# rafifmalikdzaki/Multitask-Bonetumor-yolo

Measured on AMD Instinct MI355X. Metric: images/sec at 640x640 multitask fwd (det+seg+cls) + decode/NMS/masks, higher is better.
Workload: dtype bf16; 1 GPU; configs[1]: batch-16/GPU 640x640 multitask inference (ConvNeXt-T + C2f-BiFPN + Detect/Segment/cls) + decode + per-image NMS(top-100) + mask assembly; random-init weights; batch_per_gpu=16, img=640, parallelism=dp1 (batch sharded, no data-path collective)

## Files before the change

multitask_bonetumor_yolo_amd/build.py:

```python
import os
import subprocess
import sys
from concurrent.futures import ThreadPoolExecutor

HERE = os.path.dirname(os.path.abspath(__file__))
CSRC = os.path.join(HERE, "csrc")
INCLUDE = os.path.join(os.path.dirname(HERE), "include")
LIB = os.path.join(CSRC, "libmtbt_hip.so")
SOURCES = ["conv_igemm.hip", "conv_igemm_bf16.hip", "conv_igemm_bf16_n.hip", "conv_direct_bf16.hip", "conv_igemm_f32.hip", "conv_igemm_f32_n.hip", "conv_direct_f32.hip", "conv_igemm_f16.hip", "conv_igemm_f16_n.hip", "conv_direct_f16.hip", "conv_batch_bf16.hip", "conv_batch_f16.hip", "conv_batch_f32.hip", "dwconv.hip", "dwconv_bf16.hip", "dwconv_f16.hip", "dwconv_f32.hip", "pointwise.hip", "postprocess.hip", "mask_mfma.hip", "mask_frame.hip", "bn_train.hip", "mlp_fused.hip", "upconv_fused.hip", "node_gemm.hip", "pw_stream.hip", "pw_chain.hip", "loss.hip", "mask_loss.hip", "det_loss_tal.hip", "preprocess.hip", "metrics.hip", "optim.hip", "wgrad.hip", "pointwise_bwd.hip", "train_ops.hip", "resample_bwd.hip", "box_eval.hip", "mask_eval.hip", "box_fuse.hip", "mask_vote.hip", "tile_merge.hip", "mask_tiles.hip"]
HIPCC = os.environ.get("HIPCC", "/opt/rocm/bin/hipcc")
FLAGS = ["--offload-arch=gfx950", "-O3", "-std=c++17", "-fPIC", "-I" + INCLUDE, "-I" + CSRC,
         "-fno-gpu-rdc", "-Wno-unused-value"]
if os.environ.get("MTBT_CONV_ABLATION"):
    FLAGS.append("-DMTBT_CONV_ABLATION")


EXTRA_FLAGS = {"postprocess.hip": ["-ffp-contract=off"], "loss.hip": ["-ffp-contract=off"], "mask_loss.hip": ["-ffp-contract=off"], "det_loss_tal.hip": ["-ffp-contract=off"], "preprocess.hip": ["-ffp-contract=off"], "optim.hip": ["-ffp-contract=off"],
               "box_eval.hip": ["-ffp-contract=off"], "mask_frame.hip": ["-ffp-contract=off"], "box_fuse.hip": ["-ffp-contract=off"], "mask_vote.hip": ["-ffp-contract=off"],
               "tile_merge.hip": ["-ffp-contract=off"], "mask_tiles.hip": ["-ffp-contract=off"]}


def _newer(target, deps):
    if not os.path.exists(target):
        return True
    t = os.path.getmtime(target)
    return any(os.path.getmtime(d) > t for d in deps)


def build(force: bool = False, verbose: bool = False) -> str:
    headers = [os.path.join(INCLUDE, "mtbt_hip.h")] + [os.path.join(CSRC, f) for f in os.listdir(CSRC) if f.endswith((".h", ".inc"))]
    jobs = []
    for s in SOURCES:
        src = os.path.join(CSRC, s)
        obj = os.path.join(CSRC, s.replace(".hip", ".o"))
        if force or _newer(obj, [src] + headers):
            jobs.append([HIPCC] + FLAGS + EXTRA_FLAGS.get(s, []) + ["-c", src, "-o", obj])

    def run(cmd):
        if verbose:
            print(" ".join(cmd), flush=True)
        r = subprocess.run(cmd, capture_output=True, text=True)
        if r.returncode != 0:
            raise RuntimeError("hipcc failed:\n" + " ".join(cmd) + "\n" + r.stdout + r.stderr)

    if jobs:
        with ThreadPoolExecutor(max_workers=min(8, len(jobs))) as ex:
            list(ex.map(run, jobs))
    objs = [os.path.join(CSRC, s.replace(".hip", ".o")) for s in SOURCES]
    if force or jobs or _newer(LIB, objs):
        run([HIPCC, "--offload-arch=gfx950", "-shared", "-fPIC", "-o", LIB] + objs)
    return LIB


if __name__ == "__main__":
    print(build(force="--force" in sys.argv, verbose=True))
```

multitask_bonetumor_yolo_amd/csrc/mlp_fused.hip:

```cpp
#include <cstdlib>

#include "common.h"
#include "conv_params.h"
#include "conv_dma.h"
#include "conv_epilogue.h"

namespace {

typedef __bf16 bf16x2_t __attribute__((ext_vector_type(2)));
typedef float f32x2_t __attribute__((ext_vector_type(2)));
__device__ __forceinline__ uint32_t pk_bf16(float a, float b) {
  return __builtin_bit_cast(uint32_t, __builtin_convertvector(f32x2_t{a, b}, bf16x2_t));
}

__device__ __forceinline__ f32x2_t gelu_poly2(f32x2_t x) {
  const f32x2_t xc = f32x2_t{__builtin_amdgcn_fmed3f(x.x, -4.0f, 4.0f), __builtin_amdgcn_fmed3f(x.y, -4.0f, 4.0f)};
  const f32x2_t s = xc * xc;
  auto k = [](float c) { return f32x2_t{c, c}; };
  f32x2_t p = __builtin_elementwise_fma(k(2.1609857e-08f), s, k(-1.5335673e-06f));
  p = __builtin_elementwise_fma(p, s, k(4.6542096e-05f));
  p = __builtin_elementwise_fma(p, s, k(-7.9887325e-04f));
  p = __builtin_elementwise_fma(p, s, k(8.6900834e-03f));
  p = __builtin_elementwise_fma(p, s, k(-6.4366050e-02f));
  p = __builtin_elementwise_fma(p, s, k(3.9770728e-01f));
  return x * __builtin_elementwise_fma(xc, p, k(0.5f));
}

__device__ __forceinline__ int swz4(int row) { return (-(row >> 2)) & 3; }

#ifdef MTBT_MLP_ABLATION
#define MLP_ABL(p, bit) ((p).dbg & (bit))
#else
#define MLP_ABL(p, bit) 0
#endif

#ifndef MTBT_MLP_RESIDENT
#define MTBT_MLP_RESIDENT 0
#endif

struct MlpP {
  const bf16_t* t;
  const bf16_t* w1;
  const float* b1;
  const bf16_t* w2p;
  const bf16_t* res;
  bf16_t* hpre;
  int M;
  int dbg;
  ConvP ep;
};

template <typename HT> __device__ __forceinline__ uint32_t pk2(float a, float b);
template <> __device__ __forceinline__ uint32_t pk2<bf16_t>(float a, float b) { return pk_bf16(a, b); }
template <> __device__ __forceinline__ uint32_t pk2<f16_t>(float a, float b) { return pk_h2(a, b); }
__device__ __forceinline__ int w2_row_channel(int r) {
  const int F = r >> 4, q = (r >> 2) & 3, e = r & 3;
  return 32 * (F >> 1) + 8 * q + 4 * (F & 1) + e;
}
template <typename HT> __device__ __forceinline__ f32x4 unpack4(uint2 r);
template <> __device__ __forceinline__ f32x4 unpack4<bf16_t>(uint2 r) {
  return f32x4{__uint_as_float(r.x << 16), __uint_as_float(r.x & 0xffff0000u), __uint_as_float(r.y << 16), __uint_as_float(r.y & 0xffff0000u)};
}
template <> __device__ __forceinline__ f32x4 unpack4<f16_t>(uint2 r) { return f32x4{h_lo(r.x), h_hi(r.x), h_lo(r.y), h_hi(r.y)}; }

template <int D, int FP, int WPS, typename HT, bool PIPE = false, bool HP = false>
__global__ __launch_bounds__(256, WPS) void mlp_fused_kernel(const MlpP p) {
  constexpr int KS1 = D / 32;
  constexpr int FC = D / 16;
  constexpr int NCH = 4 * D / 32;
  constexpr int PW = FP * 16, P = 4 * PW;
  constexpr int W1B = 32 * D * 2, W2B = D * 64;
  constexpr int STAGE = W1B + W2B;
  constexpr int NDMA = STAGE / 1024, DPW = NDMA / 4;
  static_assert(NDMA % 4 == 0 && W1B % 1024 == 0, "whole wave-instructions");
  constexpr int NBUF = 3;
  static_assert(NCH % NBUF == 0, "chunk loop is unrolled by the stage count");
  constexpr int AFF_OFF = NBUF * STAGE;

  extern __shared__ __attribute__((aligned(16))) char smem[];
  float* aff = reinterpret_cast<float*>(smem + AFF_OFF);
  const int tid = threadIdx.x, lane = tid & 63;
  const int wave = __builtin_amdgcn_readfirstlane(tid >> 6);
  const int lr = lane & 15, lq = lane >> 4;
  const int pbase = blockIdx.x * P + wave * PW;
  stage_affine<D>(p.ep, aff, 0, tid);
  float* b1s = aff + 2 * D;
  for (int c = tid; c < 4 * D; c += 256) b1s[c] = p.b1[c];

  const srd_t w1srd = make_srd(p.w1), w2srd = make_srd(p.w2p);
  const unsigned lds0 = (unsigned)(size_t)(__attribute__((address_space(3))) char*)smem;
  unsigned voff[DPW];
#pragma unroll
  for (int i = 0; i < DPW; ++i) {
    const int inst = i * 4 + wave;
    const int c = inst * 64 + lane;
    if (inst * 1024 < W1B) {
      const int slab = c / 128, r = (c % 128) / 4, q = (c % 4) ^ swz4(r);
      voff[i] = (unsigned)(r * D * 2 + slab * 64 + q * 16);
    } else {
      const int c2 = c - W1B / 16;
      const int r = c2 / 4, q = (c2 % 4) ^ swz4(r);
      voff[i] = (unsigned)(w2_row_channel(r) * 4 * D * 2 + q * 16);
    }
  }
  auto stage = [&](int j, int buf) {
#pragma unroll
    for (int i = 0; i < DPW; ++i) {
      const int inst = i * 4 + wave;
      const unsigned dst = lds0 + buf * STAGE + inst * 1024;
      if (inst * 1024 < W1B) lds_dma16(w1srd, voff[i], j * 32 * D * 2, dst);
      else lds_dma16(w2srd, voff[i], j * 64, dst);
    }
  };

  uint4 tf[FP][KS1];
#pragma unroll
  for (int f = 0; f < FP; ++f) {
    const int pix = pbase + f * 16 + lr;
#pragma unroll
    for (int ks = 0; ks < KS1; ++ks)
      tf[f][ks] = (pix < p.M && !(p.dbg & 64)) ? *reinterpret_cast<const uint4*>(p.t + (long)pix * D + ks * 32 + lq * 8) : uint4{0u, 0u, 0u, 0u};
  }

  f32x4 acc2[FC][FP];
  static_assert(FC % 2 == 0, "fragment pairs");
#pragma unroll
  for (int f = 0; f < FP; ++f) {
    const int pix = pbase + f * 16 + lr;
#pragma unroll
    for (int m = 0; m < FC / 2; ++m) {
      uint4 r = uint4{0u, 0u, 0u, 0u};
      if (p.res && pix < p.M) r = *reinterpret_cast<const uint4*>(p.res + (long)pix * D + m * 32 + lq * 8);
      acc2[2 * m][f] = unpack4<HT>(uint2{r.x, r.y});
      acc2[2 * m + 1][f] = unpack4<HT>(uint2{r.z, r.w});
    }
  }

  int a1off[KS1], a2off;
#pragma unroll
  for (int ks = 0; ks < KS1; ++ks) a1off[ks] = ks * 2048 + lr * 64 + ((lq ^ swz4(lr)) << 4);
  a2off = W1B + lr * 64 + ((lq ^ swz4(lr)) << 4);

  unsigned hpoff[HP ? FP : 1];
  if constexpr (HP) {
#pragma unroll
    for (int f = 0; f < FP; ++f) hpoff[f] = (unsigned)(pbase + f * 16 + lr) * (unsigned)(8 * D) + (unsigned)(lq * 16);
  }
  stage(0, 0);
  stage(1, 1);
#pragma unroll 1
  for (int j = 0; j < NCH; j += NBUF) {
#pragma unroll
    for (int u = 0; u < NBUF; ++u) {
      const int jj = j + u;
      if (jj + 1 < NCH) wait_vm<DPW + (HP ? FP : 0)>(); else wait_vm<0>();
      lds_barrier();
      if (jj + 2 < NCH && !(p.dbg & 8)) stage(jj + 2, (u + 2) % NBUF);
      const char* st = smem + u * STAGE;
      const float4 ba = *reinterpret_cast<const float4*>(b1s + jj * 32 + lq * 4);
      const float4 bb = *reinterpret_cast<const float4*>(b1s + jj * 32 + 16 + lq * 4);
      if constexpr (PIPE) {
        static_assert(FP == 2, "two pixel blocks per wave");
        uint4 hp0, hp1;
        auto gelu_half = [&](const f32x4& hv, const float4& bv, uint32_t& lo, uint32_t& hi, uint32_t& plo, uint32_t& phi) {
          f32x2_t a01 = f32x2_t{hv[0] + bv.x, hv[1] + bv.y}, a23 = f32x2_t{hv[2] + bv.z, hv[3] + bv.w};
          if constexpr (HP) { plo = pk2<HT>(a01.x, a01.y); phi = pk2<HT>(a23.x, a23.y); }
          a01 = gelu_poly2(a01); a23 = gelu_poly2(a23);
          lo = pk2<HT>(a01.x, a01.y); hi = pk2<HT>(a23.x, a23.y);
        };
        uint4 hb0, hb1;
        f32x4 h0a = f32x4{0.f, 0.f, 0.f, 0.f}, h0b = h0a, h1a = h0a, h1b = h0a;
        {
          uint4 wa[KS1];
#pragma unroll
          for (int ks = 0; ks < KS1; ++ks) wa[ks] = *reinterpret_cast<const uint4*>(st + a1off[ks]);
#pragma unroll
          for (int ks = 0; ks < KS1; ++ks) {
            h0a = mfma_16x16x32<HT>(wa[ks], tf[0][ks], h0a);
            h1a = mfma_16x16x32<HT>(wa[ks], tf[1][ks], h1a);
          }
          __builtin_amdgcn_sched_group_barrier(0x100, KS1, 0);
          __builtin_amdgcn_sched_group_barrier(0x008, 2 * KS1, 0);
        }
        __builtin_amdgcn_sched_barrier(0);
#pragma unroll
        for (int e = 0; e < 4; ++e) { asm volatile("" : "+v"(h0a[e])); asm volatile("" : "+v"(h1a[e])); }
        {
          uint4 wb[KS1];
#pragma unroll
          for (int ks = 0; ks < KS1; ++ks) wb[ks] = *reinterpret_cast<const uint4*>(st + a1off[ks] + 1024);
#pragma unroll
          for (int ks = 0; ks < KS1; ++ks) {
            h0b = mfma_16x16x32<HT>(wb[ks], tf[0][ks], h0b);
            h1b = mfma_16x16x32<HT>(wb[ks], tf[1][ks], h1b);
          }
          gelu_half(h0a, ba, hb0.x, hb0.y, hp0.x, hp0.y);
          gelu_half(h1a, ba, hb1.x, hb1.y, hp1.x, hp1.y);
          __builtin_amdgcn_sched_group_barrier(0x100, KS1, 0);
          __builtin_amdgcn_sched_group_barrier(0x006, 8, 0);
#pragma unroll
          for (int g = 0; g < 2 * KS1; ++g) {
            __builtin_amdgcn_sched_group_barrier(0x008, 1, 0);
            __builtin_amdgcn_sched_group_barrier(0x006, 6, 0);
          }
        }
        __builtin_amdgcn_sched_barrier(0);
        gelu_half(h0b, bb, hb0.z, hb0.w, hp0.z, hp0.w);
        gelu_half(h1b, bb, hb1.z, hb1.w, hp1.z, hp1.w);
        if constexpr (HP) {
          if (pbase + lr < p.M) *reinterpret_cast<uint4*>(reinterpret_cast<char*>(p.hpre) + (size_t)(jj * 64) + (size_t)hpoff[0]) = hp0;
          if (pbase + 16 + lr < p.M) *reinterpret_cast<uint4*>(reinterpret_cast<char*>(p.hpre) + (size_t)(jj * 64) + (size_t)hpoff[1]) = hp1;
        }
        constexpr int PD = 4;
        uint4 w2q[PD];
#pragma unroll
        for (int i = 0; i < PD; ++i) w2q[i] = *reinterpret_cast<const uint4*>(st + a2off + i * 1024);
#pragma unroll
        for (int i = 0; i < FC; ++i) {
          const uint4 w2 = w2q[i % PD];
          if (i + PD < FC) w2q[i % PD] = *reinterpret_cast<const uint4*>(st + a2off + (i + PD) * 1024);
          acc2[i][0] = mfma_16x16x32<HT>(w2, hb0, acc2[i][0]);
          acc2[i][1] = mfma_16x16x32<HT>(w2, hb1, acc2[i][1]);
        }
        __builtin_amdgcn_sched_group_barrier(0x100, PD, 0);
        __builtin_amdgcn_sched_group_barrier(0x006, 400, 0);
#pragma unroll
        for (int i = 0; i < FC; ++i) {
          __builtin_amdgcn_sched_group_barrier(0x008, 2, 0);
          __builtin_amdgcn_sched_group_barrier(0x100, 1, 0);
        }
      } else {
      f32x4 h[2][FP];
#pragma unroll
      for (int b = 0; b < 2; ++b)
#pragma unroll
        for (int f = 0; f < FP; ++f) h[b][f] = f32x4{0.f, 0.f, 0.f, 0.f};
      if (!(p.dbg & 4))
#pragma unroll
      for (int ks = 0; ks < KS1; ++ks) {
        const uint4 wa = *reinterpret_cast<const uint4*>(st + a1off[ks]);
        const uint4 wb = *reinterpret_cast<const uint4*>(st + a1off[ks] + 1024);
#pragma unroll
        for (int f = 0; f < FP; ++f) {
          h[0][f] = mfma_16x16x32<HT>(wa, tf[f][ks], h[0][f]);
          h[1][f] = mfma_16x16x32<HT>(wb, tf[f][ks], h[1][f]);
        }
      }
      uint4 hb[FP];
#pragma unroll
      for (int f = 0; f < FP; ++f) {
        f32x2_t a01 = f32x2_t{h[0][f][0] + ba.x, h[0][f][1] + ba.y}, a23 = f32x2_t{h[0][f][2] + ba.z, h[0][f][3] + ba.w};
        f32x2_t c01 = f32x2_t{h[1][f][0] + bb.x, h[1][f][1] + bb.y}, c23 = f32x2_t{h[1][f][2] + bb.z, h[1][f][3] + bb.w};
        if constexpr (HP) {
          if (pbase + f * 16 + lr < p.M)
            *reinterpret_cast<uint4*>(reinterpret_cast<char*>(p.hpre) + (size_t)(jj * 64) + (size_t)hpoff[f]) =
                uint4{pk2<HT>(a01.x, a01.y), pk2<HT>(a23.x, a23.y), pk2<HT>(c01.x, c01.y), pk2<HT>(c23.x, c23.y)};
        }
        if (!(p.dbg & 1)) { a01 = gelu_poly2(a01); a23 = gelu_poly2(a23); c01 = gelu_poly2(c01); c23 = gelu_poly2(c23); }
        hb[f].x = pk2<HT>(a01.x, a01.y); hb[f].y = pk2<HT>(a23.x, a23.y);
        hb[f].z = pk2<HT>(c01.x, c01.y); hb[f].w = pk2<HT>(c23.x, c23.y);
      }
      if (!(p.dbg & 2))
#pragma unroll
      for (int i = 0; i < FC; ++i) {
        const uint4 w2 = *reinterpret_cast<const uint4*>(st + a2off + i * 1024);
#pragma unroll
        for (int f = 0; f < FP; ++f)
          acc2[i][f] = mfma_16x16x32<HT>(w2, hb[f], acc2[i][f]);
      }
      }
    }
  }
  if (p.dbg & 32) { if (acc2[0][0][0] == 123.f) reinterpret_cast<bf16_t*>(p.ep.y)[0] = 0; return; }
  bf16_t* yb = reinterpret_cast<bf16_t*>(p.ep.y);
#pragma unroll
  for (int m = 0; m < FC / 2; ++m) {
    const float4 s0 = *reinterpret_cast<const float4*>(aff + D + m * 32 + lq * 8), s1 = *reinterpret_cast<const float4*>(aff + D + m * 32 + lq * 8 + 4);
#pragma unroll
    for (int f = 0; f < FP; ++f) {
      const int pix = pbase + f * 16 + lr;
      if (pix >= p.M) continue;
      u32x4 o;
      o.x = pk2<HT>(acc2[2 * m][f][0] + s0.x, acc2[2 * m][f][1] + s0.y);
      o.y = pk2<HT>(acc2[2 * m][f][2] + s0.z, acc2[2 * m][f][3] + s0.w);
      o.z = pk2<HT>(acc2[2 * m + 1][f][0] + s1.x, acc2[2 * m + 1][f][1] + s1.y);
      o.w = pk2<HT>(acc2[2 * m + 1][f][2] + s1.z, acc2[2 * m + 1][f][3] + s1.w);
      *reinterpret_cast<u32x4*>(yb + (long)pix * D + m * 32 + lq * 8) = o;
    }
  }
}

template <int D, int FP, int WPS, typename HT, bool PIPE = false, bool HP = false>
int launch_mlp(const MlpP& p, hipStream_t s) {
  constexpr int P = 4 * FP * 16;
  constexpr int STAGE = 32 * D * 2 + D * 64;
  constexpr int lds = 3 * STAGE + 2 * D * 4 + 4 * D * 4;
  static_assert(lds <= 160 * 1024, "LDS");
  const long blocks = ((long)p.M + P - 1) / P;
  if (blocks <= 0 || blocks > 0x7fffffffL) return MTBT_EINVAL;
  if (int rc = mtbt_allow_lds(mlp_fused_kernel<D, FP, WPS, HT, PIPE, HP>, lds)) return rc;
  hipLaunchKernelGGL((mlp_fused_kernel<D, FP, WPS, HT, PIPE, HP>), dim3((unsigned)blocks), dim3(256), lds, s, p);
  MTBT_LAUNCH_CHECK();
  return MTBT_OK;
}


template <int D, typename HT, bool ORD = false, bool HP = false>
__global__ __launch_bounds__(512, 2) void mlp_pair_kernel(const MlpP p) {
  constexpr int FP = 2;
  constexpr int KS1 = D / 32, FCH = D / 32, NCH = 4 * D / 32;
  constexpr int PW = FP * 16, P = 4 * PW;
  constexpr int W1B = 32 * D * 2, W2B = D * 64, STAGE = W1B + W2B;
  constexpr int NDMA = STAGE / 1024, DPW = NDMA / 8;
  static_assert(NDMA % 8 == 0 && W1B % 1024 == 0, "whole wave-instructions per wave");
  constexpr int XCH_OFF = 2 * STAGE, XCH_BYTES = 2 * 4 * 2 * FP * 64 * 8;
  constexpr int AFF_OFF = XCH_OFF + XCH_BYTES;
  extern __shared__ __attribute__((aligned(16))) char smem[];
  float* aff = reinterpret_cast<float*>(smem + AFF_OFF);
  float* b1s = aff + D;
  const int tid = threadIdx.x, lane = tid & 63;
  const int wave = __builtin_amdgcn_readfirstlane(tid >> 6);
  const int g = wave >> 1, hh = wave & 1;
  const int lr = lane & 15, lq = lane >> 4;
  const int pbase = blockIdx.x * P + g * PW;
  for (int c = tid; c < D; c += 512) aff[c] = p.ep.shift[c];
  for (int c = tid; c < 4 * D; c += 512) b1s[c] = p.b1[c];

  const srd_t w1srd = make_srd(p.w1), w2srd = make_srd(p.w2p);
  const unsigned lds0 = (unsigned)(size_t)(__attribute__((address_space(3))) char*)smem;
  unsigned voff[DPW];
#pragma unroll
  for (int i = 0; i < DPW; ++i) {
    const int inst = i * 8 + wave;
    const int c = inst * 64 + lane;
    if (inst * 1024 < W1B) {
      const int slab = c / 128, r = (c % 128) / 4, sl = (c % 4) ^ swz4(r);
      voff[i] = (unsigned)(r * D * 2 + slab * 64 + sl * 16);
    } else {
      const int c2 = c - W1B / 16;
      const int r = c2 / 4, sl = (c2 % 4) ^ swz4(r);
      voff[i] = (unsigned)(w2_row_channel(r) * 4 * D * 2 + sl * 16);
    }
  }
  auto stage = [&](int j, int buf) {
#pragma unroll
    for (int i = 0; i < DPW; ++i) {
      const int inst = i * 8 + wave;
      const unsigned dst = lds0 + buf * STAGE + inst * 1024;
      if (inst * 1024 < W1B) { if (j < NCH) lds_dma16(w1srd, voff[i], j * 32 * D * 2, dst); }
      else { if (j >= 1) lds_dma16(w2srd, voff[i], (j - 1) * 64, dst); }
    }
  };

  uint4 tf[FP][KS1];
  f32x4 acc2[FCH][FP];
#pragma unroll
  for (int f = 0; f < FP; ++f) {
    const int pix = pbase + f * 16 + lr;
#pragma unroll
    for (int ks = 0; ks < KS1; ++ks)
      tf[f][ks] = (pix < p.M && !MLP_ABL(p, 64)) ? *reinterpret_cast<const uint4*>(p.t + (long)pix * D + ks * 32 + lq * 8) : uint4{0u, 0u, 0u, 0u};
#pragma unroll
    for (int m = 0; m < FCH / 2; ++m) {
      uint4 r = uint4{0u, 0u, 0u, 0u};
      if (p.res && pix < p.M) r = *reinterpret_cast<const uint4*>(p.res + (long)pix * D + (hh * FCH / 2 + m) * 32 + lq * 8);
      acc2[2 * m][f] = unpack4<HT>(uint2{r.x, r.y});
      acc2[2 * m + 1][f] = unpack4<HT>(uint2{r.z, r.w});
    }
  }
  int a1off[KS1];
#pragma unroll
  for (int ks = 0; ks < KS1; ++ks) a1off[ks] = ks * 2048 + hh * 1024 + lr * 64 + ((lq ^ swz4(lr)) << 4);
  const int a2off = W1B + (hh * FCH * 16 + lr) * 64 + ((lq ^ swz4(lr)) << 4);
  uint2* const xch = reinterpret_cast<uint2*>(smem + XCH_OFF);
  const int xmine = ((g * 2 + hh) * FP) * 64 + lane, xpeer = ((g * 2 + (1 - hh)) * FP) * 64 + lane;

  auto gemm2 = [&](const char* st, const uint4 (&hb)[FP]) {
    if (MLP_ABL(p, 2)) return;
#pragma unroll
    for (int i = 0; i < FCH; ++i) {
      const uint4 w2 = *reinterpret_cast<const uint4*>(st + a2off + i * 1024);
#pragma unroll
      for (int f = 0; f < FP; ++f) acc2[i][f] = mfma_16x16x32<HT>(w2, hb[f], acc2[i][f]);
    }
  };
  const bool ord = ORD && (wave & 4);
  uint2 mine[FP];
#pragma unroll
  for (int f = 0; f < FP; ++f) mine[f] = uint2{0u, 0u};
  unsigned hpoff[HP ? FP : 1];
  if constexpr (HP) {
#pragma unroll
    for (int f = 0; f < FP; ++f) hpoff[f] = (unsigned)(pbase + f * 16 + lr) * (unsigned)(8 * D) + (unsigned)(lq * 16 + hh * 8);
  }
  stage(0, 0);
#pragma unroll 1
  for (int j0 = 0; j0 <= NCH; j0 += 2) {
#pragma unroll
    for (int u = 0; u < 2; ++u) {
      const int j = j0 + u;
      if (j > NCH) break;
      wait_vm<0>();
      lds_barrier();
      if (j + 1 <= NCH && !MLP_ABL(p, 8)) stage(j + 1, (u + 1) & 1);
      const char* st = smem + u * STAGE;
      uint4 hb[FP];
      if (j >= 1) {
#pragma unroll
        for (int f = 0; f < FP; ++f) {
          const uint2 peer = xch[((u + 1) & 1) * (4 * 2 * FP * 64) + xpeer + f * 64];
          hb[f] = hh == 0 ? uint4{mine[f].x, mine[f].y, peer.x, peer.y} : uint4{peer.x, peer.y, mine[f].x, mine[f].y};
        }
      }
      f32x4 h[FP];
      const bool g2_first = ord && j >= 1;
      if (g2_first) gemm2(st, hb);
      if (j < NCH) {
#pragma unroll
        for (int f = 0; f < FP; ++f) h[f] = f32x4{0.f, 0.f, 0.f, 0.f};
        if (!MLP_ABL(p, 4))
#pragma unroll
        for (int ks = 0; ks < KS1; ++ks) {
          const uint4 w = *reinterpret_cast<const uint4*>(st + a1off[ks]);
#pragma unroll
          for (int f = 0; f < FP; ++f) h[f] = mfma_16x16x32<HT>(w, tf[f][ks], h[f]);
        }
      }
      if (j >= 1 && !g2_first) gemm2(st, hb);
      if (j < NCH) {
        const float4 bv = *reinterpret_cast<const float4*>(b1s + j * 32 + hh * 16 + lq * 4);
#pragma unroll
        for (int f = 0; f < FP; ++f) {
          f32x2_t a01 = f32x2_t{h[f][0] + bv.x, h[f][1] + bv.y}, a23 = f32x2_t{h[f][2] + bv.z, h[f][3] + bv.w};
          if constexpr (HP) {
            if (pbase + f * 16 + lr < p.M)
              *reinterpret_cast<uint2*>(reinterpret_cast<char*>(p.hpre) + (size_t)(j * 64) + (size_t)hpoff[f]) = uint2{pk2<HT>(a01.x, a01.y), pk2<HT>(a23.x, a23.y)};
          }
          if (!MLP_ABL(p, 1)) { a01 = gelu_poly2(a01); a23 = gelu_poly2(a23); }
          mine[f] = uint2{pk2<HT>(a01.x, a01.y), pk2<HT>(a23.x, a23.y)};
          xch[u * (4 * 2 * FP * 64) + xmine + f * 64] = mine[f];
        }
      }
    }
  }
  HT* const yb = reinterpret_cast<HT*>(p.ep.y);
  static_assert(FCH % 2 == 0, "fragment pairs");
#pragma unroll
  for (int m = 0; m < FCH / 2; ++m) {
    const int cb = (hh * FCH / 2 + m) * 32 + lq * 8;
    const float4 s0 = *reinterpret_cast<const float4*>(aff + cb), s1 = *reinterpret_cast<const float4*>(aff + cb + 4);
#pragma unroll
    for (int f = 0; f < FP; ++f) {
      const int pix = pbase + f * 16 + lr;
      if (pix >= p.M || MLP_ABL(p, 32)) continue;
      u32x4 o;
      o.x = pk2<HT>(acc2[2 * m][f][0] + s0.x, acc2[2 * m][f][1] + s0.y);
      o.y = pk2<HT>(acc2[2 * m][f][2] + s0.z, acc2[2 * m][f][3] + s0.w);
      o.z = pk2<HT>(acc2[2 * m + 1][f][0] + s1.x, acc2[2 * m + 1][f][1] + s1.y);
      o.w = pk2<HT>(acc2[2 * m + 1][f][2] + s1.z, acc2[2 * m + 1][f][3] + s1.w);
      *reinterpret_cast<u32x4*>(yb + (long)pix * D + cb) = o;
    }
  }
}

template <int D, typename HT, bool ORD = false, bool HP = false>
int launch_mlp_pair(const MlpP& p, hipStream_t s) {
  constexpr int P = 4 * 2 * 16;
  constexpr int STAGE = 32 * D * 2 + D * 64;
  constexpr int lds = 2 * STAGE + 2 * 4 * 2 * 2 * 64 * 8 + 5 * D * 4;
  static_assert(lds <= 160 * 1024, "LDS");
  const long blocks = ((long)p.M + P - 1) / P;
  if (blocks <= 0 || blocks > 0x7fffffffL) return MTBT_EINVAL;
  if (int rc = mtbt_allow_lds(mlp_pair_kernel<D, HT, ORD, HP>, lds)) return rc;
  hipLaunchKernelGGL((mlp_pair_kernel<D, HT, ORD, HP>), dim3((unsigned)blocks), dim3(512), lds, s, p);
  MTBT_LAUNCH_CHECK();
  return MTBT_OK;
}

template <int D, typename HT, int NW, bool PREF = false>
__global__ __launch_bounds__(NW * 64, NW / 4) void mlp_resident_kernel(const MlpP p) {
  constexpr int FP = 2;
  constexpr int KS1 = D / 32, FC = D / 16, NCH = 4 * D / 32;
  constexpr int W1B = 32 * D * 2, W2B = D * 64, STAGE = W1B + W2B;
  static_assert(NCH * STAGE + 6 * D * 4 <= 160 * 1024, "the weights must fit the LDS");
  extern __shared__ __attribute__((aligned(16))) char smem[];
  float* aff = reinterpret_cast<float*>(smem + NCH * STAGE);
  float* b1s = aff + D;
  const int tid = threadIdx.x, lane = tid & 63;
  const int wave = __builtin_amdgcn_readfirstlane(tid >> 6);
  const int lr = lane & 15, lq = lane >> 4;
  for (int c = tid; c < D; c += NW * 64) aff[c] = p.ep.shift[c];
  for (int c = tid; c < 4 * D; c += NW * 64) b1s[c] = p.b1[c];
  {
    const srd_t w1srd = make_srd(p.w1), w2srd = make_srd(p.w2p);
    const unsigned lds0 = (unsigned)(size_t)(__attribute__((address_space(3))) char*)smem;
    constexpr int NDMA = STAGE / 1024;
    for (int q = wave; q < NCH * NDMA; q += NW) {
      const int j = q / NDMA, inst = q - j * NDMA;
      const int c = inst * 64 + lane;
      unsigned vo;
      if (inst * 1024 < W1B) {
        const int slab = c / 128, r = (c % 128) / 4, sl = (c % 4) ^ swz4(r);
        vo = (unsigned)(r * D * 2 + slab * 64 + sl * 16);
        lds_dma16(w1srd, vo, j * 32 * D * 2, __builtin_amdgcn_readfirstlane(lds0 + j * STAGE + inst * 1024));
      } else {
        const int c2 = c - W1B / 16;
        const int r = c2 / 4, sl = (c2 % 4) ^ swz4(r);
        vo = (unsigned)(r * 4 * D * 2 + sl * 16);
        lds_dma16(w2srd, vo, j * 64, __builtin_amdgcn_readfirstlane(lds0 + j * STAGE + inst * 1024));
      }
    }
    wait_vm<0>();
  }
  __syncthreads();

  int a1off[KS1], a2off;
#pragma unroll
  for (int ks = 0; ks < KS1; ++ks) a1off[ks] = ks * 2048 + lr * 64 + ((lq ^ swz4(lr)) << 4);
  a2off = W1B + lr * 64 + ((lq ^ swz4(lr)) << 4);

  const int nblk = (p.M + 31) / 32;
  const int G = gridDim.x, per_round = G * NW;
  const int rounds = nblk / per_round, rem = nblk - rounds * per_round;
  const int mine = rounds + ((wave * G + (int)blockIdx.x) < rem ? 1 : 0);
  HT* const yb = reinterpret_cast<HT*>(p.ep.y);
  auto block_of = [&](int it) { return it < rounds ? it * per_round + (int)blockIdx.x * NW + wave : rounds * per_round + wave * G + (int)blockIdx.x; };
  auto fetch = [&](int blk, uint4 (&tf_)[FP][KS1], uint2 (&rr_)[FC][FP]) {
#pragma unroll
    for (int f = 0; f < FP; ++f) {
      const int pix = blk * 32 + f * 16 + lr;
#pragma unroll
      for (int ks = 0; ks < KS1; ++ks)
        tf_[f][ks] = (pix < p.M && !MLP_ABL(p, 64)) ? *reinterpret_cast<const uint4*>(p.t + (unsigned)(pix * D + ks * 32 + lq * 8)) : uint4{0u, 0u, 0u, 0u};
#pragma unroll
      for (int i = 0; i < FC; ++i)
        rr_[i][f] = (p.res && pix < p.M) ? *reinterpret_cast<const uint2*>(p.res + (unsigned)(pix * D + i * 16 + lq * 4)) : uint2{0u, 0u};
    }
  };
  uint4 tf[FP][KS1], tfn[FP][KS1];
  uint2 rr[FC][FP], rrn[FC][FP];
  if (PREF && mine > 0) fetch(block_of(0), tf, rr);
#pragma unroll 1
  for (int it = 0; it < mine; ++it) {
    const int blk = block_of(it);
    const int pbase = blk * 32;
    if (PREF) { if (it + 1 < mine) fetch(block_of(it + 1), tfn, rrn); }
    else fetch(blk, tf, rr);
    f32x4 acc2[FC][FP];
#pragma unroll
    for (int f = 0; f < FP; ++f)
#pragma unroll
      for (int i = 0; i < FC; ++i) acc2[i][f] = unpack4<HT>(rr[i][f]);
#pragma unroll 1
    for (int jj = 0; jj < NCH; ++jj) {
      const char* st = smem + jj * STAGE;
      const float4 ba = *reinterpret_cast<const float4*>(b1s + jj * 32 + lq * 4);
      const float4 bb = *reinterpret_cast<const float4*>(b1s + jj * 32 + 16 + lq * 4);
      f32x4 h[2][FP];
#pragma unroll
      for (int b = 0; b < 2; ++b)
#pragma unroll
        for (int f = 0; f < FP; ++f) h[b][f] = f32x4{0.f, 0.f, 0.f, 0.f};
      if (!MLP_ABL(p, 4))
#pragma unroll
      for (int ks = 0; ks < KS1; ++ks) {
        const uint4 wa = *reinterpret_cast<const uint4*>(st + a1off[ks]);
        const uint4 wb = *reinterpret_cast<const uint4*>(st + a1off[ks] + 1024);
#pragma unroll
        for (int f = 0; f < FP; ++f) {
          h[0][f] = mfma_16x16x32<HT>(wa, tf[f][ks], h[0][f]);
          h[1][f] = mfma_16x16x32<HT>(wb, tf[f][ks], h[1][f]);
        }
      }
      uint4 hb[FP];
#pragma unroll
      for (int f = 0; f < FP; ++f) {
        f32x2_t a01 = f32x2_t{h[0][f][0] + ba.x, h[0][f][1] + ba.y}, a23 = f32x2_t{h[0][f][2] + ba.z, h[0][f][3] + ba.w};
        f32x2_t c01 = f32x2_t{h[1][f][0] + bb.x, h[1][f][1] + bb.y}, c23 = f32x2_t{h[1][f][2] + bb.z, h[1][f][3] + bb.w};
        if (!MLP_ABL(p, 1)) { a01 = gelu_poly2(a01); a23 = gelu_poly2(a23); c01 = gelu_poly2(c01); c23 = gelu_poly2(c23); }
        hb[f].x = pk2<HT>(a01.x, a01.y); hb[f].y = pk2<HT>(a23.x, a23.y);
        hb[f].z = pk2<HT>(c01.x, c01.y); hb[f].w = pk2<HT>(c23.x, c23.y);
      }
      if (!MLP_ABL(p, 2))
#pragma unroll
      for (int i = 0; i < FC; ++i) {
        const uint4 w2 = *reinterpret_cast<const uint4*>(st + a2off + i * 1024);
#pragma unroll
        for (int f = 0; f < FP; ++f) acc2[i][f] = mfma_16x16x32<HT>(w2, hb[f], acc2[i][f]);
      }
    }
#pragma unroll
    for (int i = 0; i < FC; ++i) {
      const float4 sh = *reinterpret_cast<const float4*>(aff + i * 16 + lq * 4);
#pragma unroll
      for (int f = 0; f < FP; ++f) {
        const int pix = pbase + f * 16 + lr;
        if (pix >= p.M || MLP_ABL(p, 32)) continue;
        uint2 o;
        o.x = pk2<HT>(acc2[i][f][0] + sh.x, acc2[i][f][1] + sh.y);
        o.y = pk2<HT>(acc2[i][f][2] + sh.z, acc2[i][f][3] + sh.w);
        *reinterpret_cast<uint2*>(yb + (unsigned)(pix * D + i * 16 + lq * 4)) = o;
      }
    }
    if (PREF) {
#pragma unroll
      for (int f = 0; f < FP; ++f) {
#pragma unroll
        for (int ks = 0; ks < KS1; ++ks) tf[f][ks] = tfn[f][ks];
#pragma unroll
        for (int i = 0; i < FC; ++i) rr[i][f] = rrn[i][f];
      }
    }
  }
}

template <int D, typename HT, int NW = 16, bool PREF = false>
int launch_mlp_resident(const MlpP& p, hipStream_t s) {
  constexpr int lds = (4 * D / 32) * (32 * D * 2 + D * 64) + 5 * D * 4;
  const long nblk = ((long)p.M + 31) / 32;
  long blocks = (nblk + NW - 1) / NW;
  if (blocks > 256) blocks = 256;
  if (blocks <= 0) return MTBT_EINVAL;
  if (int rc = mtbt_allow_lds(mlp_resident_kernel<D, HT, NW, PREF>, lds)) return rc;
  hipLaunchKernelGGL((mlp_resident_kernel<D, HT, NW, PREF>), dim3((unsigned)blocks), dim3(NW * 64), lds, s, p);
  MTBT_LAUNCH_CHECK();
  return MTBT_OK;
}

}

static int mlp_entry(const void* t, const void* res, const void* w1, const float* b1, const void* w2p, const float* b2, void* y, int64_t M, int D,
                     int dtype, void* stream, void* hpre = nullptr) {
  if (!t || !w1 || !b1 || !w2p || !b2 || !y || M <= 0 || M > 0x7fffff00L) return MTBT_EINVAL;
  if (hpre && (dtype != MTBT_BF16 || !aligned16(hpre) || M * 8 * (int64_t)D >= 0xffff0000L)) return MTBT_EINVAL;
  if (dtype != MTBT_BF16 && dtype != MTBT_F16) return MTBT_EINVAL;
  if (D != 96 && D != 192 && D != 384) return MTBT_EINVAL;
  if (!aligned16(t) || !aligned16(w1) || !aligned16(w2p) || !aligned16(y) || !aligned16(b1) || (res && !aligned16(res))) return MTBT_EALIGN;
  if ((long)4 * D * D * 2 >= 0x7fff0000L) return MTBT_EINVAL;
  MlpP p;
  p.t = reinterpret_cast<const bf16_t*>(t); p.w1 = reinterpret_cast<const bf16_t*>(w1); p.b1 = b1;
  p.w2p = reinterpret_cast<const bf16_t*>(w2p); p.M = (int)M;
  p.dbg = 0;
  p.hpre = reinterpret_cast<bf16_t*>(hpre);
  ConvP& e = p.ep;
  e = ConvP{};
  p.res = (p.dbg & 16) ? nullptr : reinterpret_cast<const bf16_t*>(res);
  e.y = y; e.res = nullptr;
  e.scale = nullptr; e.shift = b2; e.K = D; e.ldy = D; e.ldr = D; e.act = MTBT_ACT_NONE;
  e.out_mode = MTBT_OUT_NHWC; e.out_f32 = 0; e.vec_ok = 1; e.M = (int)M;
  hipStream_t s = reinterpret_cast<hipStream_t>(stream);
  if (D == 96 && M >= 64 * 1024 && M * 96 < 0x7fffffffL && MTBT_MLP_RESIDENT)
    return dtype == MTBT_F16 ? launch_mlp_resident<96, f16_t, 8, true>(p, s) : launch_mlp_resident<96, bf16_t, 8, true>(p, s);
  if (hpre) {
    if (D == 384) return MTBT_EINVAL;
    if (D == 192) return launch_mlp<192, 2, 2, bf16_t, true, true>(p, s);
    return launch_mlp<96, 2, 4, bf16_t, false, true>(p, s);
  }
  if (D == 384) return dtype == MTBT_F16 ? launch_mlp_pair<384, f16_t>(p, s) : launch_mlp_pair<384, bf16_t>(p, s);
  if (D == 192) return dtype == MTBT_F16 ? launch_mlp<192, 2, 2, f16_t, true>(p, s) : launch_mlp<192, 2, 2, bf16_t, true>(p, s);
  return dtype == MTBT_F16 ? launch_mlp<96, 2, 4, f16_t>(p, s) : launch_mlp<96, 2, 4, bf16_t>(p, s);
}

extern "C" int mtbt_convnext_mlp_fused(const void* t, const void* res, const void* w1, const float* b1, const void* w2p,
                                       const float* b2, void* y, int64_t M, int D, void* stream) {
  return mlp_entry(t, res, w1, b1, w2p, b2, y, M, D, MTBT_BF16, stream);
}

extern "C" int mtbt_convnext_mlp_fused_dt(const void* t, const void* res, const void* w1, const float* b1, const void* w2p,
                                          const float* b2, void* y, int64_t M, int D, int dtype, void* stream) {
  return mlp_entry(t, res, w1, b1, w2p, b2, y, M, D, dtype, stream);
}

extern "C" int mtbt_convnext_mlp_fused_train(const void* t, const void* res, const void* w1_perm, const float* b1_perm, const void* w2, const float* b2,
                                             void* y, void* hpre, int64_t M, int D, void* stream) {
  if (!hpre) return MTBT_EINVAL;
  return mlp_entry(t, res, w1_perm, b1_perm, w2, b2, y, M, D, MTBT_BF16, stream, hpre);
}
```

Before: 2707 images/s.

## Deepen mlp_pair weight ring and interleave GELU with GEMM2 MFMAs

The pair MLP kernel gains a RING=3 default mode in which W1 chunks are triple-buffered and W2' chunks double-buffered in LDS, so staging runs further ahead of compute and uses partial vmcnt waits. GELU is split into staged pieces that are interleaved with the GEMM2 MFMA steps, and LDS weight fragments are prefetched a couple of steps ahead, with sched_barriers pinning the order. The aim is to hide DMA latency and VALU GELU work behind matrix instructions. In exchange it uses more LDS per block, which may reduce occupancy, adds register pressure, and makes the scheduling fragile. The build also compiles a test probe library.

Measured after the change: 2742 images/s (median of 6 runs). Within noise of the previous version (+1.3%).

```diff
diff --git a/multitask_bonetumor_yolo_amd/build.py b/multitask_bonetumor_yolo_amd/build.py
--- a/multitask_bonetumor_yolo_amd/build.py
+++ b/multitask_bonetumor_yolo_amd/build.py
@@ -8,6 +8,8 @@
 INCLUDE = os.path.join(os.path.dirname(HERE), "include")
 LIB = os.path.join(CSRC, "libmtbt_hip.so")
 SOURCES = ["conv_igemm.hip", "conv_igemm_bf16.hip", "conv_igemm_bf16_n.hip", "conv_direct_bf16.hip", "conv_igemm_f32.hip", "conv_igemm_f32_n.hip", "conv_direct_f32.hip", "conv_igemm_f16.hip", "conv_igemm_f16_n.hip", "conv_direct_f16.hip", "conv_batch_bf16.hip", "conv_batch_f16.hip", "conv_batch_f32.hip", "dwconv.hip", "dwconv_bf16.hip", "dwconv_f16.hip", "dwconv_f32.hip", "pointwise.hip", "postprocess.hip", "mask_mfma.hip", "mask_frame.hip", "bn_train.hip", "mlp_fused.hip", "upconv_fused.hip", "node_gemm.hip", "pw_stream.hip", "pw_chain.hip", "loss.hip", "mask_loss.hip", "det_loss_tal.hip", "preprocess.hip", "metrics.hip", "optim.hip", "wgrad.hip", "pointwise_bwd.hip", "train_ops.hip", "resample_bwd.hip", "box_eval.hip", "mask_eval.hip", "box_fuse.hip", "mask_vote.hip", "tile_merge.hip", "mask_tiles.hip"]
+PROBES = os.path.join(os.path.dirname(HERE), "tools", "probes")
+TEST_PROBES = ["mlp_pair_ring"]
 HIPCC = os.environ.get("HIPCC", "/opt/rocm/bin/hipcc")
 FLAGS = ["--offload-arch=gfx950", "-O3", "-std=c++17", "-fPIC", "-I" + INCLUDE, "-I" + CSRC,
          "-fno-gpu-rdc", "-Wno-unused-value"]
@@ -27,8 +29,30 @@
     return any(os.path.getmtime(d) > t for d in deps)
 
 
+def _headers():
+    return [os.path.join(INCLUDE, "mtbt_hip.h")] + [os.path.join(CSRC, f) for f in os.listdir(CSRC) if f.endswith((".h", ".inc"))]
+
+
+def _probe_job(name, force):
+    src = os.path.join(PROBES, name + ".hip")
+    lib = os.path.join(PROBES, "lib" + name + ".so")
+    deps = [src] + _headers() + [os.path.join(CSRC, f) for f in os.listdir(CSRC) if f.endswith(".hip")]
+    cmd = [HIPCC] + FLAGS + ["-shared", src, "-o", lib] if force or _newer(lib, deps) else None
+    return lib, cmd
+
+
+def build_probe(name: str, force: bool = False) -> str:
+    lib, cmd = _probe_job(name, force)
+    if cmd:
+        r = subprocess.run(cmd, capture_output=True, text=True)
+        if r.returncode != 0:
+            raise RuntimeError("hipcc failed:\n" + " ".join(cmd) + "\n" + r.stdout + r.stderr)
+    return lib
+
+
 def build(force: bool = False, verbose: bool = False) -> str:
-    headers = [os.path.join(INCLUDE, "mtbt_hip.h")] + [os.path.join(CSRC, f) for f in os.listdir(CSRC) if f.endswith((".h", ".inc"))]
+    headers = _headers()
+    probes = [cmd for _, cmd in (_probe_job(n, force) for n in TEST_PROBES) if cmd]
     jobs = []
     for s in SOURCES:
         src = os.path.join(CSRC, s)
@@ -43,9 +67,9 @@
         if r.returncode != 0:
             raise RuntimeError("hipcc failed:\n" + " ".join(cmd) + "\n" + r.stdout + r.stderr)
 
-    if jobs:
-        with ThreadPoolExecutor(max_workers=min(8, len(jobs))) as ex:
-            list(ex.map(run, jobs))
+    if jobs or probes:
+        with ThreadPoolExecutor(max_workers=min(8, len(jobs) + len(probes))) as ex:
+            list(ex.map(run, probes + jobs))
     objs = [os.path.join(CSRC, s.replace(".hip", ".o")) for s in SOURCES]
     if force or jobs or _newer(LIB, objs):
         run([HIPCC, "--offload-arch=gfx950", "-shared", "-fPIC", "-o", LIB] + objs)
diff --git a/multitask_bonetumor_yolo_amd/csrc/mlp_fused.hip b/multitask_bonetumor_yolo_amd/csrc/mlp_fused.hip
--- a/multitask_bonetumor_yolo_amd/csrc/mlp_fused.hip
+++ b/multitask_bonetumor_yolo_amd/csrc/mlp_fused.hip
@@ -1,4 +1,5 @@
 #include <cstdlib>
+#include <type_traits>
 
 #include "common.h"
 #include "conv_params.h"
@@ -13,17 +14,24 @@
   return __builtin_bit_cast(uint32_t, __builtin_convertvector(f32x2_t{a, b}, bf16x2_t));
 }
 
+struct GeluSt { f32x2_t x, xc, s, p; };
+constexpr int GELU_STAGES = 10;
+__device__ __forceinline__ void gelu_poly2_stage(GeluSt& g, int st) {
+  constexpr float C[7] = {2.1609857e-08f, -1.5335673e-06f, 4.6542096e-05f, -7.9887325e-04f, 8.6900834e-03f, -6.4366050e-02f, 3.9770728e-01f};
+  auto k = [](float c) { return f32x2_t{c, c}; };
+  if (st == 0) g.xc = f32x2_t{__builtin_amdgcn_fmed3f(g.x.x, -4.0f, 4.0f), __builtin_amdgcn_fmed3f(g.x.y, -4.0f, 4.0f)};
+  else if (st == 1) g.s = g.xc * g.xc;
+  else if (st == 2) g.p = __builtin_elementwise_fma(k(C[0]), g.s, k(C[1]));
+  else if (st <= 7) g.p = __builtin_elementwise_fma(g.p, g.s, k(C[st - 1]));
+  else if (st == 8) g.p = __builtin_elementwise_fma(g.xc, g.p, k(0.5f));
+  else g.x = g.x * g.p;
+}
 __device__ __forceinline__ f32x2_t gelu_poly2(f32x2_t x) {
-  const f32x2_t xc = f32x2_t{__builtin_amdgcn_fmed3f(x.x, -4.0f, 4.0f), __builtin_amdgcn_fmed3f(x.y, -4.0f, 4.0f)};
-  const f32x2_t s = xc * xc;
-  auto k = [](float c) { return f32x2_t{c, c}; };
-  f32x2_t p = __builtin_elementwise_fma(k(2.1609857e-08f), s, k(-1.5335673e-06f));
-  p = __builtin_elementwise_fma(p, s, k(4.6542096e-05f));
-  p = __builtin_elementwise_fma(p, s, k(-7.9887325e-04f));
-  p = __builtin_elementwise_fma(p, s, k(8.6900834e-03f));
-  p = __builtin_elementwise_fma(p, s, k(-6.4366050e-02f));
-  p = __builtin_elementwise_fma(p, s, k(3.9770728e-01f));
-  return x * __builtin_elementwise_fma(xc, p, k(0.5f));
+  GeluSt g;
+  g.x = x;
+#pragma unroll
+  for (int st = 0; st < GELU_STAGES; ++st) gelu_poly2_stage(g, st);
+  return g.x;
 }
 
 __device__ __forceinline__ int swz4(int row) { return (-(row >> 2)) & 3; }
@@ -305,7 +313,14 @@
 }
 
 
-template <int D, typename HT, bool ORD = false, bool HP = false>
+template <int D, int RING> constexpr int mlp_pair_lds() {
+  constexpr int W1B = 32 * D * 2, W2B = D * 64;
+  return (RING == 2 ? 2 * (W1B + W2B) : 3 * W1B + 2 * W2B) + 2 * 4 * 2 * 2 * 64 * 8 + 5 * D * 4;
+}
+template <int BASE> __device__ __forceinline__ void wait_vm_plus(int k) {
+  if (k <= 0) wait_vm<BASE>(); else if (k == 1) wait_vm<BASE + 1>(); else wait_vm<BASE + 2>();
+}
+template <int D, typename HT, bool ORD = false, bool HP = false, int RING = 3>
 __global__ __launch_bounds__(512, 2) void mlp_pair_kernel(const MlpP p) {
   constexpr int FP = 2;
   constexpr int KS1 = D / 32, FCH = D / 32, NCH = 4 * D / 32;
@@ -313,8 +328,12 @@
   constexpr int W1B = 32 * D * 2, W2B = D * 64, STAGE = W1B + W2B;
   constexpr int NDMA = STAGE / 1024, DPW = NDMA / 8;
   static_assert(NDMA % 8 == 0 && W1B % 1024 == 0, "whole wave-instructions per wave");
-  constexpr int XCH_OFF = 2 * STAGE, XCH_BYTES = 2 * 4 * 2 * FP * 64 * 8;
+  static_assert(RING == 2 || RING == 3, "two whole stages, or W1 three deep and W2' two deep");
+  static_assert(!ORD || RING == 2, "the opposite phase order exists in the two-stage form only");
+  constexpr int W1_OFF = 0, W1_STEP = RING == 2 ? STAGE : W1B, W2_OFF = RING == 2 ? W1B : 3 * W1B, W2_STEP = RING == 2 ? STAGE : W2B;
+  constexpr int XCH_OFF = RING == 2 ? 2 * STAGE : 3 * W1B + 2 * W2B, XCH_BYTES = 2 * 4 * 2 * FP * 64 * 8;
   constexpr int AFF_OFF = XCH_OFF + XCH_BYTES;
+  static_assert(AFF_OFF + 5 * D * 4 == mlp_pair_lds<D, RING>() && mlp_pair_lds<D, RING>() <= 160 * 1024, "LDS budget");
   extern __shared__ __attribute__((aligned(16))) char smem[];
   float* aff = reinterpret_cast<float*>(smem + AFF_OFF);
   float* b1s = aff + D;
@@ -323,8 +342,11 @@
   const int g = wave >> 1, hh = wave & 1;
   const int lr = lane & 15, lq = lane >> 4;
   const int pbase = blockIdx.x * P + g * PW;
-  for (int c = tid; c < D; c += 512) aff[c] = p.ep.shift[c];
-  for (int c = tid; c < 4 * D; c += 512) b1s[c] = p.b1[c];
+  auto fill_bias = [&]() {
+    for (int c = tid; c < D; c += 512) aff[c] = p.ep.shift[c];
+    for (int c = tid; c < 4 * D; c += 512) b1s[c] = p.b1[c];
+  };
+  if constexpr (RING == 2) fill_bias();
 
   const srd_t w1srd = make_srd(p.w1), w2srd = make_srd(p.w2p);
   const unsigned lds0 = (unsigned)(size_t)(__attribute__((address_space(3))) char*)smem;
@@ -351,6 +373,19 @@
       else { if (j >= 1) lds_dma16(w2srd, voff[i], (j - 1) * 64, dst); }
     }
   };
+  constexpr int DW = W1B / 1024 / 8;
+  static_assert(RING == 2 || ((W1B / 1024) % 8 == 0 && DPW == 2 * DW), "every wave stages DW pieces of W1 and DW of W2'");
+  auto stage_w1 = [&](int chunk, int off) {
+#pragma unroll
+    for (int i = 0; i < DW; ++i) lds_dma16(w1srd, voff[0], chunk * 32 * D * 2 + i * 4 * 64, lds0 + off + (i * 8 + wave) * 1024);
+  };
+  auto stage_w2 = [&](int chunk, int off) {
+#pragma unroll
+    for (int i = 0; i < DW; ++i) lds_dma16(w2srd, voff[DW], chunk * 64 + i * 128 * 4 * D * 2, lds0 + off + (i * 8 + wave) * 1024);
+  };
+  if constexpr (RING == 3) {
+    stage_w1(0, W1_OFF); stage_w1(1, W1_OFF + W1_STEP);
+  }
 
   uint4 tf[FP][KS1];
   f32x4 acc2[FCH][FP];
@@ -368,10 +403,11 @@
       acc2[2 * m + 1][f] = unpack4<HT>(uint2{r.z, r.w});
     }
   }
+  if constexpr (RING == 3) fill_bias();
   int a1off[KS1];
 #pragma unroll
   for (int ks = 0; ks < KS1; ++ks) a1off[ks] = ks * 2048 + hh * 1024 + lr * 64 + ((lq ^ swz4(lr)) << 4);
-  const int a2off = W1B + (hh * FCH * 16 + lr) * 64 + ((lq ^ swz4(lr)) << 4);
+  const int a2off = (hh * FCH * 16 + lr) * 64 + ((lq ^ swz4(lr)) << 4);
   uint2* const xch = reinterpret_cast<uint2*>(smem + XCH_OFF);
   const int xmine = ((g * 2 + hh) * FP) * 64 + lane, xpeer = ((g * 2 + (1 - hh)) * FP) * 64 + lane;
 
@@ -393,55 +429,154 @@
 #pragma unroll
     for (int f = 0; f < FP; ++f) hpoff[f] = (unsigned)(pbase + f * 16 + lr) * (unsigned)(8 * D) + (unsigned)(lq * 16 + hh * 8);
   }
-  stage(0, 0);
+  if constexpr (RING == 2) {
+    stage(0, 0);
 #pragma unroll 1
-  for (int j0 = 0; j0 <= NCH; j0 += 2) {
-#pragma unroll
-    for (int u = 0; u < 2; ++u) {
-      const int j = j0 + u;
-      if (j > NCH) break;
-      wait_vm<0>();
+    for (int j0 = 0; j0 <= NCH; j0 += 2) {
+#pragma unroll
+      for (int u = 0; u < 2; ++u) {
+        const int j = j0 + u;
+        if (j > NCH) break;
+        wait_vm<0>();
+        lds_barrier();
+        if (j + 1 <= NCH && !MLP_ABL(p, 8)) stage(j + 1, (u + 1) & 1);
+        const char* st = smem + u * STAGE;
+        uint4 hb[FP];
+        if (j >= 1) {
+#pragma unroll
+          for (int f = 0; f < FP; ++f) {
+            const uint2 peer = xch[((u + 1) & 1) * (4 * 2 * FP * 64) + xpeer + f * 64];
+            hb[f] = hh == 0 ? uint4{mine[f].x, mine[f].y, peer.x, peer.y} : uint4{peer.x, peer.y, mine[f].x, mine[f].y};
+          }
+        }
+        f32x4 h[FP];
+        const bool g2_first = ord && j >= 1;
+        if (g2_first) gemm2(st + W2_OFF, hb);
+        if (j < NCH) {
+#pragma unroll
+          for (int f = 0; f < FP; ++f) h[f] = f32x4{0.f, 0.f, 0.f, 0.f};
+          if (!MLP_ABL(p, 4))
+#pragma unroll
+          for (int ks = 0; ks < KS1; ++ks) {
+            const uint4 w = *reinterpret_cast<const uint4*>(st + a1off[ks]);
+#pragma unroll
+            for (int f = 0; f < FP; ++f) h[f] = mfma_16x16x32<HT>(w, tf[f][ks], h[f]);
+          }
+        }
+        if (j >= 1 && !g2_first) gemm2(st + W2_OFF, hb);
+        if (j < NCH) {
+          const float4 bv = *reinterpret_cast<const float4*>(b1s + j * 32 + hh * 16 + lq * 4);
+#pragma unroll
+          for (int f = 0; f < FP; ++f) {
+            f32x2_t a01 = f32x2_t{h[f][0] + bv.x, h[f][1] + bv.y}, a23 = f32x2_t{h[f][2] + bv.z, h[f][3] + bv.w};
+            if constexpr (HP) {
+              if (pbase + f * 16 + lr < p.M)
+                *reinterpret_cast<uint2*>(reinterpret_cast<char*>(p.hpre) + (size_t)(j * 64) + (size_t)hpoff[f]) = uint2{pk2<HT>(a01.x, a01.y), pk2<HT>(a23.x, a23.y)};
+            }
+            if (!MLP_ABL(p, 1)) { a01 = gelu_poly2(a01); a23 = gelu_poly2(a23); }
+            mine[f] = uint2{pk2<HT>(a01.x, a01.y), pk2<HT>(a23.x, a23.y)};
+            xch[u * (4 * 2 * FP * 64) + xmine + f * 64] = mine[f];
+          }
+        }
+      }
+    }
+  } else {
+    const int nst = HP ? __builtin_amdgcn_readfirstlane((pbase < p.M ? 1 : 0) + (pbase + 16 < p.M ? 1 : 0)) : 0;
+    constexpr int XP = 4 * 2 * FP * 64;
+    auto iter = [&](auto first_, auto last_, const int j, const int w1rd, const int w1wr) {
+      constexpr bool FIRST = decltype(first_)::value, LAST = decltype(last_)::value;
+      const int par = j & 1;
+      if constexpr (FIRST) wait_vm<0>();
+      else if (!LAST && j + 1 < NCH && !MLP_ABL(p, 128)) wait_vm_plus<DW>(nst);
+      else wait_vm_plus<0>(nst);
       lds_barrier();
-      if (j + 1 <= NCH && !MLP_ABL(p, 8)) stage(j + 1, (u + 1) & 1);
-      const char* st = smem + u * STAGE;
-      uint4 hb[FP];
-      if (j >= 1) {
-#pragma unroll
-        for (int f = 0; f < FP; ++f) {
-          const uint2 peer = xch[((u + 1) & 1) * (4 * 2 * FP * 64) + xpeer + f * 64];
-          hb[f] = hh == 0 ? uint4{mine[f].x, mine[f].y, peer.x, peer.y} : uint4{peer.x, peer.y, mine[f].x, mine[f].y};
-        }
-      }
+      if constexpr (!LAST) {
+        if (!MLP_ABL(p, 8)) {
+          stage_w2(j, W2_OFF + (par ^ 1) * W2_STEP);
+          if (j + 2 < NCH) stage_w1(j + 2, w1wr);
+        }
+      }
+      constexpr int PD = 2;
+      const char* const s1 = smem + W1_OFF + w1rd;
+      const char* const s2 = smem + W2_OFF + par * W2_STEP + a2off;
       f32x4 h[FP];
-      const bool g2_first = ord && j >= 1;
-      if (g2_first) gemm2(st, hb);
-      if (j < NCH) {
+      uint4 wq[PD];
+      uint2 peer[FP], own[FP];
+      float4 bv;
+      if constexpr (!FIRST) {
+#pragma unroll
+        for (int f = 0; f < FP; ++f) { peer[f] = xch[(par ^ 1) * XP + xpeer + f * 64]; own[f] = xch[(par ^ 1) * XP + xmine + f * 64]; }
+      }
+      if constexpr (!LAST) {
+        bv = *reinterpret_cast<const float4*>(b1s + j * 32 + hh * 16 + lq * 4);
+#pragma unroll
+        for (int i = 0; i < PD; ++i) wq[i] = *reinterpret_cast<const uint4*>(s1 + a1off[i]);
+      }
+      __builtin_amdgcn_sched_barrier(0);
+      if constexpr (!LAST) {
 #pragma unroll
         for (int f = 0; f < FP; ++f) h[f] = f32x4{0.f, 0.f, 0.f, 0.f};
-        if (!MLP_ABL(p, 4))
 #pragma unroll
         for (int ks = 0; ks < KS1; ++ks) {
-          const uint4 w = *reinterpret_cast<const uint4*>(st + a1off[ks]);
-#pragma unroll
-          for (int f = 0; f < FP; ++f) h[f] = mfma_16x16x32<HT>(w, tf[f][ks], h[f]);
-        }
-      }
-      if (j >= 1 && !g2_first) gemm2(st, hb);
-      if (j < NCH) {
-        const float4 bv = *reinterpret_cast<const float4*>(b1s + j * 32 + hh * 16 + lq * 4);
-#pragma unroll
-        for (int f = 0; f < FP; ++f) {
-          f32x2_t a01 = f32x2_t{h[f][0] + bv.x, h[f][1] + bv.y}, a23 = f32x2_t{h[f][2] + bv.z, h[f][3] + bv.w};
+          if (!MLP_ABL(p, 4)) {
+            const uint4 w = wq[ks % PD];
+#pragma unroll
+            for (int f = 0; f < FP; ++f) h[f] = mfma_16x16x32<HT>(w, tf[f][ks], h[f]);
+          }
+          if (ks + PD < KS1) wq[ks % PD] = *reinterpret_cast<const uint4*>(s1 + a1off[ks + PD]);
+          else if constexpr (!FIRST) wq[ks % PD] = *reinterpret_cast<const uint4*>(s2 + (ks + PD - KS1) * 1024);
+          __builtin_amdgcn_sched_barrier(0);
+        }
+      } else {
+#pragma unroll
+        for (int i = 0; i < PD; ++i) wq[i] = *reinterpret_cast<const uint4*>(s2 + i * 1024);
+      }
+      constexpr int GSTEPS = GELU_STAGES + 2;
+      static_assert(FP * GSTEPS == 2 * FCH, "two GELU pieces beside every step of GEMM2");
+      GeluSt ga, gb;
+      auto gelu_piece = [&](int f, int st) {
+        if (st == 0) {
+          ga.x = f32x2_t{h[f][0] + bv.x, h[f][1] + bv.y}; gb.x = f32x2_t{h[f][2] + bv.z, h[f][3] + bv.w};
           if constexpr (HP) {
             if (pbase + f * 16 + lr < p.M)
-              *reinterpret_cast<uint2*>(reinterpret_cast<char*>(p.hpre) + (size_t)(j * 64) + (size_t)hpoff[f]) = uint2{pk2<HT>(a01.x, a01.y), pk2<HT>(a23.x, a23.y)};
+              *reinterpret_cast<uint2*>(reinterpret_cast<char*>(p.hpre) + (size_t)(j * 64) + (size_t)hpoff[f]) = uint2{pk2<HT>(ga.x.x, ga.x.y), pk2<HT>(gb.x.x, gb.x.y)};
           }
-          if (!MLP_ABL(p, 1)) { a01 = gelu_poly2(a01); a23 = gelu_poly2(a23); }
-          mine[f] = uint2{pk2<HT>(a01.x, a01.y), pk2<HT>(a23.x, a23.y)};
-          xch[u * (4 * 2 * FP * 64) + xmine + f * 64] = mine[f];
-        }
-      }
-    }
+        } else if (st <= GELU_STAGES) {
+          if (!MLP_ABL(p, 1)) { gelu_poly2_stage(ga, st - 1); gelu_poly2_stage(gb, st - 1); }
+        } else {
+          xch[par * XP + xmine + f * 64] = uint2{pk2<HT>(ga.x.x, ga.x.y), pk2<HT>(gb.x.x, gb.x.y)};
+        }
+      };
+      if constexpr (!FIRST) {
+        uint4 hb[FP];
+#pragma unroll
+        for (int f = 0; f < FP; ++f)
+          hb[f] = hh == 0 ? uint4{own[f].x, own[f].y, peer[f].x, peer[f].y} : uint4{peer[f].x, peer[f].y, own[f].x, own[f].y};
+#pragma unroll
+        for (int i = 0; i < FCH; ++i) {
+          if (!MLP_ABL(p, 2)) {
+            const uint4 w = wq[i % PD];
+#pragma unroll
+            for (int f = 0; f < FP; ++f) acc2[i][f] = mfma_16x16x32<HT>(w, hb[f], acc2[i][f]);
+          }
+          if (i + PD < FCH) wq[i % PD] = *reinterpret_cast<const uint4*>(s2 + (i + PD) * 1024);
+          if constexpr (!LAST) { gelu_piece(2 * i / GSTEPS, 2 * i % GSTEPS); gelu_piece(2 * i / GSTEPS, 2 * i % GSTEPS + 1); }
+          __builtin_amdgcn_sched_barrier(0);
+        }
+      } else {
+#pragma unroll
+        for (int g2 = 0; g2 < FP * GSTEPS; ++g2) gelu_piece(g2 / GSTEPS, g2 % GSTEPS);
+      }
+    };
+    auto next_slot = [](int off) { return off == 2 * W1_STEP ? 0 : off + W1_STEP; };
+    iter(std::true_type{}, std::false_type{}, 0, 0, 2 * W1_STEP);
+    int w1rd = W1_STEP, w1wr = 0;
+#pragma unroll 1
+    for (int j = 1; j < NCH; ++j) {
+      iter(std::false_type{}, std::false_type{}, j, w1rd, w1wr);
+      w1rd = next_slot(w1rd); w1wr = next_slot(w1wr);
+    }
+    iter(std::false_type{}, std::true_type{}, NCH, 0, 0);
   }
   HT* const yb = reinterpret_cast<HT*>(p.ep.y);
   static_assert(FCH % 2 == 0, "fragment pairs");
@@ -463,16 +598,15 @@
   }
 }
 
-template <int D, typename HT, bool ORD = false, bool HP = false>
+template <int D, typename HT, bool ORD = false, bool HP = false, int RING = 3>
 int launch_mlp_pair(const MlpP& p, hipStream_t s) {
   constexpr int P = 4 * 2 * 16;
-  constexpr int STAGE = 32 * D * 2 + D * 64;
-  constexpr int lds = 2 * STAGE + 2 * 4 * 2 * 2 * 64 * 8 + 5 * D * 4;
+  constexpr int lds = mlp_pair_lds<D, RING>();
   static_assert(lds <= 160 * 1024, "LDS");
   const long blocks = ((long)p.M + P - 1) / P;
   if (blocks <= 0 || blocks > 0x7fffffffL) return MTBT_EINVAL;
-  if (int rc = mtbt_allow_lds(mlp_pair_kernel<D, HT, ORD, HP>, lds)) return rc;
-  hipLaunchKernelGGL((mlp_pair_kernel<D, HT, ORD, HP>), dim3((unsigned)blocks), dim3(512), lds, s, p);
+  if (int rc = mtbt_allow_lds(mlp_pair_kernel<D, HT, ORD, HP, RING>, lds)) return rc;
+  hipLaunchKernelGGL((mlp_pair_kernel<D, HT, ORD, HP, RING>), dim3((unsigned)blocks), dim3(512), lds, s, p);
   MTBT_LAUNCH_CHECK();
   return MTBT_OK;
 }
```
